# nash169/manifold-gp

Hardware: AMD Instinct MI355X
Metric: CG-solve wall-time + SpMV HBM GB/s, N=60k RMNIST graph (higher is better)
Workload: dtype f32; 1 GPU; C3 RMNIST-like N=60000 d=784 k=50 nu=2 randomwalk; nodes=60000, edges=1777442, nnz_padded=3667592, rhs_columns=1, system=A = I + noise*outputscale*Q, Q=(2nu/kappa^2 I + L)^nu x D, solver=CG on A (Chronopoulos-Gear, one hipGraph per solve)

## Files before the change

### include/mgp_hip.h

```cpp
#ifndef MGP_HIP_H
#define MGP_HIP_H

#include <stddef.h>
#include <stdint.h>

#ifdef __cplusplus
extern "C" {
#endif

#define MGP_OK 0
#define MGP_ERR_ARG (-1)
#define MGP_ERR_WORKSPACE (-2)
#define MGP_ERR_UNSUPPORTED (-3)
#define MGP_ERR_NOT_CONVERGED (-4)
#define MGP_ERR_KNN_AMBIGUOUS (-5)
#define MGP_ERR_TIMEOUT (-6)

#define MGP_PAD 4

int mgp_version(void);
int mgp_device_info(int* cu_count, int* wave_size, size_t* hbm_bytes);

size_t mgp_knn_workspace_bytes(int64_t N, int64_t n, int d, int k);
int mgp_knn_search(const float* db, int64_t N, int d, const float* q, int64_t n, int k,
// ... 46 lines not shown
int mgp_spmm_backward_sums(int64_t n, int C, const float* h, const float* dlx, const float* xs, const float* gxs, const float* X,
                           const float* g, const float* lx, float av, float bv, float cov, float* partial, float* gpre,
                           float* gpost, void* stream);
int mgp_edge_values(const int32_t* tri_row, const int32_t* tri_col, const float* tri_val,
                    int64_t M, const float* degree_unnorm, const float* degree, float eps,
                    int which, float* out, void* stream);

typedef struct {
  int64_t n;
  const int32_t* rowptr;
  const int32_t* col;
  const float* vals;
  const float* diag;
  int64_t ncols;
  const int32_t* tile_ptr;
  const int32_t* tile_cols;
  const uint16_t* lid;
  int32_t tile_rows;
  int32_t tile_max_cols;
  int32_t tile_max_entries;
  int32_t spmv_lanes;
  const int32_t* tile_rowptr;
  const float* tile_vals;
  const int32_t* tile_rowid;
  const int32_t* mt_sptr;
  const int32_t* mt_dcol;
  const float* mt_img;
  int32_t mt_tiles;
  int32_t mt_steps;
} mgp_csr_t;

int mgp_spmm_dot_blocks_csr(const mgp_csr_t* L, int C);
int mgp_spmm_set_tile_mode(int on);
int mgp_spmm_set_tile_small_mode(int on);
int mgp_spmm_set_tile_wide_mode(int on);
int mgp_spmm_set_dict_mode(int on);
int mgp_spmm_set_mt_mode(int on);
int mgp_spmm_kernel_choice(const mgp_csr_t* L, int C, int with_dot, int64_t row_offset);
int mgp_spmm_mt_fill(int64_t n, const int32_t* rowptr, const float* vals, const uint16_t* lid16, const int32_t* tile_ptr16,
                     const int32_t* tile_cols16, const int32_t* sptr, int64_t steps, int32_t* dcol, float* img, void* stream);
int mgp_spmm_timing_begin(int max_launches);
int mgp_spmm_timing_end(float* total_ms, int* launches);
int mgp_spmm_set_v4_mode(int on);

int mgp_spmm_dot_blocks(int64_t n, int C);
int mgp_spmm_set_group_hint(int lanes);
int mgp_spmm_set_rows_in_flight(int rows);
int mgp_spmm_fused(const mgp_csr_t* L, const float* X, int C, float* Y, float a, float b,
                   const float* pre, const float* post, const float* base, float cb, float co,
                   const float* dotw, float* dot_partials, void* stream);

int mgp_spmm_fused_rows(const mgp_csr_t* L_local, int64_t row_offset, const float* X, int C, float* Y,
                        float a, float b, const float* pre, const float* post, const float* base,
                        float cb, float co, const float* dotw, float* dot_partials, void* stream);

int mgp_spmm_repeat(const mgp_csr_t* L, const float* X, int C, float* Y, int reps, float* elapsed_ms,
                    void* stream);

int mgp_laplacian_matmul(const mgp_csr_t* L, const float* dsqrt, const float* dinvsqrt, int mode,
                         const float* X, int C, float* Y, float* work_nc, void* stream);

int mgp_gmrf_noise(const mgp_csr_t* L, const float* dsqrt, float node_coef, int tag, int with_edges,
                   uint64_t seed, int64_t sample_offset, int S, float* Y, void* stream);

typedef struct {
  mgp_csr_t L;
// ... 189 lines not shown
```

### manifold_gp_amd/_lib.py

```python
import ctypes
import os
import threading
from ctypes import (POINTER, Structure, byref, c_double, c_float, c_int, c_int32, c_int64, c_size_t,
                    c_uint64, c_void_p)

import torch

_HERE = os.path.dirname(os.path.abspath(__file__))
LIB_PATH = os.path.join(_HERE, "libmgp_hip.so")
_LIB = None
_LOCK = threading.Lock()

MGP_ERRORS = {
    -1: "MGP_ERR_ARG (null pointer / bad size / bad enum)",
    -2: "MGP_ERR_WORKSPACE (work buffer too small)",
    -3: "MGP_ERR_UNSUPPORTED",
    -4: "MGP_ERR_NOT_CONVERGED",
    -5: "MGP_ERR_KNN_AMBIGUOUS",
}


class MgpError(RuntimeError):
    def __init__(self, fn, code):
        self.code = code
# ... 26 lines not shown
class LanczosParamsT(Structure):
    _fields_ = [("max_basis", c_int32), ("degree", c_int32), ("max_restarts", c_int32),
                ("tol", c_float), ("seed", c_uint64)]


_P = c_void_p
SIGNATURES = {
    "mgp_version": (c_int, []),
    "mgp_device_info": (c_int, [POINTER(c_int), POINTER(c_int), POINTER(c_size_t)]),
    "mgp_knn_workspace_bytes": (c_size_t, [c_int64, c_int64, c_int, c_int]),
    "mgp_knn_search": (c_int, [_P, c_int64, c_int, _P, c_int64, c_int, _P, _P, _P, c_size_t,
                               POINTER(c_int64), _P]),
    "mgp_knn_set_mfma": (c_int, [c_int]),
    "mgp_knn_set_symmetric": (c_int, [c_int]),
    "mgp_knn_set_filter": (c_int, [c_int]),
    "mgp_knn_last_filter_failover": (c_int64, []),
    "mgp_knn_index_bytes": (c_size_t, [c_int64, c_int]),
    "mgp_knn_index_build": (c_int, [_P, c_int64, c_int, _P, c_size_t, _P]),
    "mgp_knn_search_indexed": (c_int, [_P, c_int64, c_int, _P, c_size_t, _P, c_int64, c_int, _P, _P, _P, c_size_t, _P, _P]),
    "mgp_knn_last_direct_chunks": (c_int64, []),
    "mgp_graph_workspace_bytes": (c_size_t, [c_int64, c_int]),
    "mgp_graph_edges": (c_int, [_P, _P, c_int64, c_int, c_int, c_int, _P, _P, _P, POINTER(c_int64), _P, c_size_t, _P]),
    "mgp_graph_tiles_workspace_bytes": (c_size_t, [c_int64, c_int64]),
    "mgp_graph_tiles": (c_int, [c_int64, _P, _P, c_int64, c_int, _P, _P, _P, _P, _P, _P, POINTER(c_int64),
                                POINTER(c_int32), POINTER(c_int32), _P, c_size_t, _P]),
    "mgp_morton_order_workspace_bytes": (c_size_t, [c_int64]),
    "mgp_morton_order": (c_int, [_P, c_int64, c_int, _P, _P, c_size_t, _P]),
    "mgp_graph_chain_order": (c_int, [c_int64, _P, _P, _P, _P, _P]),
    "mgp_permute_rows": (c_int, [_P, _P, c_int64, c_int, _P, _P]),
    "mgp_graph_bfs_workspace_bytes": (c_size_t, [c_int64]),
    "mgp_graph_bfs_order": (c_int, [c_int64, _P, _P, _P, _P, c_size_t, _P]),
    "mgp_spmm_dot_blocks_csr": (c_int, [POINTER(CsrT), c_int]),
    "mgp_spmm_set_tile_mode": (c_int, [c_int]),
    "mgp_spmm_set_tile_small_mode": (c_int, [c_int]),
    "mgp_spmm_set_tile_wide_mode": (c_int, [c_int]),
    "mgp_spmm_set_dict_mode": (c_int, [c_int]),
    "mgp_spmm_set_mt_mode": (c_int, [c_int]),
    "mgp_spmm_kernel_choice": (c_int, [POINTER(CsrT), c_int, c_int, c_int64]),
    "mgp_spmm_mt_fill": (c_int, [c_int64, _P, _P, _P, _P, _P, _P, c_int64, _P, _P, _P]),
    "mgp_spmm_timing_begin": (c_int, [c_int]),
    "mgp_spmm_timing_end": (c_int, [POINTER(c_float), POINTER(c_int)]),
    "mgp_spmm_set_v4_mode": (c_int, [c_int]),
    "mgp_cg_set_decide_in_update": (c_int, [c_int]),
    "mgp_cg_set_complex_shift": (c_int, [c_int]),
    "mgp_cg_plan_is_complex_shift": (c_int, [_P]),
    "mgp_cg_set_fold_update": (c_int, [c_int]),
    "mgp_cg_plan_is_folded": (c_int, [_P]),
    "mgp_cg_set_reduce_once": (c_int, [c_int]),
    "mgp_cg_set_update_quads": (c_int, [c_int]),
    "mgp_cg_set_poll_spin": (c_int, [c_int]),
    "mgp_cg_set_init_free": (c_int, [c_int]),
    "mgp_host_symeig": (c_int, [c_int, _P, _P, _P]),
    "mgp_lanczos_set_bound_mode": (c_int, [c_int]),
    "mgp_blz_workspace_bytes": (c_size_t, [c_int64, c_int, c_int]),
    "mgp_blz_begin": (c_int, [_P, c_int64, c_int, c_int, _P, c_size_t, _P]),
    "mgp_blz_q": (c_void_p, [c_int64, c_int, c_int, c_int, _P, c_size_t]),
    "mgp_blz_step": (c_int, [_P, c_int64, c_int, c_int, c_int, _P, c_size_t, _P]),
    "mgp_blz_end": (c_int, [c_int64, c_int, c_int, POINTER(c_float), POINTER(c_float), _P, c_size_t, _P]),
    "mgp_lanczos_tridiag_block_workspace_bytes": (c_size_t, [POINTER(OperatorT), c_int, c_int]),
    "mgp_lanczos_tridiag_block": (c_int, [POINTER(OperatorT), _P, c_int, c_int, POINTER(c_float), POINTER(c_float), _P,
                                         c_size_t, _P]),
    "mgp_graph_build": (c_int, [_P, _P, c_int64, c_int, _P, _P, _P, POINTER(c_int64), _P, _P, _P, _P,
                                POINTER(c_int64), _P, c_size_t, _P]),
    "mgp_graph_coo_workspace_bytes": (c_size_t, [c_int64, c_int64]),
    "mgp_graph_from_coo": (c_int, [_P, _P, _P, c_int64, c_int64, _P, _P, _P, _P, POINTER(c_int64), _P,
                                   c_size_t, _P]),
# ... 211 lines not shown
```

### manifold_gp_amd/csrc/spmm.hip

```cpp
#include <string.h>
#include <atomic>
#include <type_traits>
#include "mgp_common.h"
#include "mgp_internal.h"
#include "cg_rule.h"
#include "cg_handoff.h"
#include <hip/hip_ext.h>
#include <vector>

namespace {

constexpr int kBlock = 256;
constexpr int kMaxGrid = 4096;

struct SpmmArgs {
  int64_t n;
  const int32_t* rowptr;
  const int32_t* col;
  const float* vals;
  const float* diag;
  const float* X;
  float* Y;
  int C;
  float a, b;
// ... 128 lines not shown
      p.Y[myr + p.goff] = y;
      dsum = fmaf(e_dotw, y, dsum);
    }
  }
  if (p.dot_partials) {
    __shared__ float red[BS / MGP_WAVE];
    dsum = mgp_wave_sum(dsum);
    if ((threadIdx.x & 63) == 0) red[threadIdx.x >> 6] = dsum;
    __syncthreads();
    if (threadIdx.x == 0) {
      float t = 0.f;
#pragma unroll
      for (int w = 0; w < BS / MGP_WAVE; ++w) t += red[w];
      p.dot_partials[lb] = t;
    }
  }
}

struct TileArgs {
  const int32_t* tile_ptr;
  const int32_t* tile_cols;
  const uint16_t* lid;
  int64_t ntiles;
  int tiles_per_block;
  int max_cols;
  const int32_t* rowptr_t;
  const float* vals_t;
  const int32_t* rowid;
  int max_entries;
  int part_window;
};

typedef unsigned short mgp_v4h __attribute__((ext_vector_type(4)));

enum { kTilePlain = 0, kTileSelfDot = 1, kTileCgStep = 2 };
struct NoCgStep {};

template <bool PRE, int BS, bool CBV, int MODE, bool DECIDE, int DS, class CS>
__device__ __forceinline__ void spmv_tile_body(const SpmmArgs p, const TileArgs t, const CS cs) {
  extern __shared__ __attribute__((aligned(16))) float tile_lds[];
  const int lane0 = __builtin_amdgcn_mbcnt_lo(0u, 0u);
  const int* __restrict__ skip_ptr = (p.skip ? p.skip : reinterpret_cast<const int*>(p.rowptr)) + lane0;
  const int* __restrict__ tick_ptr = (p.tick ? p.tick : reinterpret_cast<const int*>(p.rowptr)) + lane0;
  int skipl = 0, tickl = 0;
  constexpr int TR = BS / 4;
  constexpr int NQ = 4;
  const int lb = mgp_xcd_block(blockIdx.x, gridDim.x);
  const int tid = threadIdx.x, sub = tid & 3;
#ifdef MGP_STAMP
  int* st_base = !p.stamp_on ? nullptr : (p.skip ? const_cast<int*>(p.skip) - 1 : p.tick);
  if (st_base && blockIdx.x == 0 && tid == 0) {
    const int si = atomicAdd(st_base + 8, 1);
    reinterpret_cast<unsigned long long*>(st_base + 16)[si & 255] = wall_clock64() * 8 + 0;
  }
  if (st_base && tid == 0 && blockIdx.x < 2048) reinterpret_cast<unsigned long long*>(st_base + 16)[256 + 2 * blockIdx.x] = wall_clock64();
#endif
  float* __restrict__ xl = tile_lds;
  float* __restrict__ part = tile_lds + t.max_cols;
  const float* __restrict__ x = p.X;
  const float* __restrict__ prev = p.pre;
  const int32_t* __restrict__ rowptr = t.rowptr_t ? t.rowptr_t : p.rowptr;
  const float* __restrict__ vals = t.vals_t ? t.vals_t : p.vals;
  const int32_t* __restrict__ tile_ptr = t.tile_ptr;
  const uint32_t* __restrict__ tile_cols = reinterpret_cast<const uint32_t*>(t.tile_cols);
  const uint16_t* __restrict__ lid = t.lid;
  float dsum = 0.f, dsum2 = 0.f;
  const int64_t t0 = (int64_t)lb * t.tiles_per_block;
  const int64_t t1 = t0 + t.tiles_per_block < t.ntiles ? t0 + t.tiles_per_block : t.ntiles;
  __shared__ float cg_sh_w[MODE == kTileCgStep ? BS / MGP_WAVE : 1][3];
  __shared__ float cg_sh_o[MODE == kTileCgStep ? BS / MGP_WAVE : 1];
  __shared__ int cg_sh_state[MODE == kTileCgStep ? 2 : 1];
  __shared__ int cg_sh_last[1];
  [[maybe_unused]] float cg_rv[2][DS], cg_dv[DS];
  [[maybe_unused]] float cg_go0 = 0.f, cg_go1 = 0.f, cg_ao0 = 0.f, cg_ao1 = 0.f, cg_bb_old = 0.f;
  [[maybe_unused]] int cg_st_it = 0, cg_st_done = 0;
  [[maybe_unused]] float cg_alpha = 0.f, cg_beta = 0.f, cg_bb = 0.f, cg_nrr = 0.f;
  [[maybe_unused]] int cg_it = 0;
  [[maybe_unused]] bool cg_fresh = false;
  if constexpr (MODE == kTileCgStep) {
    static_assert(BS == 256, "the step's sums are written for four waves");
    const CgScalars sc = *reinterpret_cast<const CgScalars*>(cs.blk);
    cg_go0 = sc.go0; cg_go1 = sc.go1; cg_ao0 = sc.ao0; cg_ao1 = sc.ao1; cg_bb_old = sc.bb; cg_st_it = sc.it; cg_st_done = sc.done;
#pragma unroll
    for (int q = 0; q < DS; ++q) {
      const int b = tid + q * BS;
      const int bc = b < cs.nbs ? b : cs.nbs - 1;
      cg_rv[0][q] = cs.pd_rr[bc];
      cg_rv[1][q] = cs.pd_rr[cs.nbs + bc];
      cg_dv[q] = cs.pd_delta[bc];
    }
  }
  for (int64_t tile = t0; tile < t1; ++tile) {
    skipl = *skip_ptr;
    tickl = *tick_ptr;
    const int64_t r0 = tile * TR;
    const int64_t r1 = r0 + TR < p.n ? r0 + TR : p.n;
    const int e0 = rowptr[r0], e1 = rowptr[r1];
    const int dp = tile_ptr[tile];
    const int D = tile_ptr[tile + 1] - dp;
    const int qb = e0 >> 2, Q = (e1 - e0) >> 2;
    unsigned c[NQ];
#pragma unroll
    for (int k = 0; k < NQ; ++k) {
      const int j = tid + k * BS;
      c[k] = (unsigned)tile_cols[j < D ? dp + j : 0];
    }
    __builtin_amdgcn_sched_barrier(0);
    mgp_v4f v[NQ];
    mgp_v4h l[NQ];
#pragma unroll
    for (int k = 0; k < NQ / 2; ++k) {
      const int q = tid + k * BS;
      const int qi = q < Q ? qb + q : 0;
      v[k] = *reinterpret_cast<const mgp_v4f*>(vals + 4 * (int64_t)qi);
      l[k] = *reinterpret_cast<const mgp_v4h*>(lid + 4 * (int64_t)qi);
    }
    __builtin_amdgcn_sched_barrier(0);
    float g[NQ];
#pragma unroll
    for (int k = 0; k < NQ; ++k) {
      g[k] = x[c[k]];
      if (PRE) g[k] *= prev[c[k]];
    }
    __builtin_amdgcn_sched_barrier(0);
#pragma unroll
    for (int k = NQ / 2; k < NQ; ++k) {
      const int q = tid + k * BS;
      const int qi = q < Q ? qb + q : 0;
      v[k] = *reinterpret_cast<const mgp_v4f*>(vals + 4 * (int64_t)qi);
      l[k] = *reinterpret_cast<const mgp_v4h*>(lid + 4 * (int64_t)qi);
    }
    __builtin_amdgcn_sched_barrier(0);
    const int64_t row = r0 + (tid >> 2);
    const bool valid = row < r1;
    const int64_t pr = valid ? row : r0;
    const int64_t rr = t.rowid ? (int64_t)t.rowid[pr] : pr;
    const int64_t grr = rr + p.goff;
    const int rs = rowptr[pr], re = rowptr[pr + 1];
    const float raw_x = x[grr];
    float e_x = raw_x;
    if (PRE) e_x *= prev[grr];
    const float e_diag = p.diag[rr];
    const float l_post = (p.post ? p.post : x)[grr], l_base = (p.base ? p.base : x)[grr], l_dotw = (p.dotw ? p.dotw : x)[grr];
    const float e_post = p.post ? l_post : 1.f;
    const float e_base = p.base ? l_base : 0.f;
    const float e_dotw = p.dotw ? l_dotw : 0.f;
    const float e_cb = CBV ? p.cbv[grr] : p.cb;
    [[maybe_unused]] float f_r = 0.f, f_s = 0.f, f_p = 0.f, f_x = 0.f, f_pre = 1.f;
    if constexpr (MODE == kTileCgStep) {
      f_r = cs.r[grr]; f_s = cs.s[grr]; f_p = cs.p[grr]; f_x = cs.x[grr];
      const float l_pre = (cs.us ? cs.pre : x)[grr];
      f_pre = cs.us ? l_pre : 1.f;
    }
    __builtin_amdgcn_sched_barrier(0);
    if (p.skip && skipl) return;
    if constexpr (MODE == kTileCgStep) {
      if (tile == t0) {
        float s3[3] = {0.f, 0.f, 0.f};
#pragma unroll
        for (int q = 0; q < DS; ++q) {
          const bool on = tid + q * BS < cs.nbs;
          s3[0] += on ? cg_rv[0][q] : 0.f; s3[1] += on ? cg_rv[1][q] : 0.f; s3[2] += on ? cg_dv[q] : 0.f;
        }
#pragma unroll
        for (int k = 0; k < 3; ++k) s3[k] = mgp_wave_sum(s3[k]);
        if ((tid & 63) == 0) {
#pragma unroll
          for (int k = 0; k < 3; ++k) cg_sh_w[tid >> 6][k] = s3[k];
        }
        if (tid == 0) { cg_sh_state[0] = cg_st_it; cg_sh_state[1] = cg_st_done; }
      }
    }
#pragma unroll
    for (int k = 0; k < NQ; ++k) {
      const int j = tid + k * BS;
      if (j < D) xl[j] = g[k];
    }
    for (int j = tid + NQ * BS; j < D; j += BS) {
      const int cc = tile_cols[dp + j];
      float gg = x[cc];
      if (PRE) gg *= prev[cc];
      xl[j] = gg;
    }
    __syncthreads();
    if constexpr (MODE == kTileCgStep) {
      if (tile == t0) {
        const int it = cg_sh_state[0];
        const bool fresh = it == 1;
        auto zero_x = [&]() {
          for (int64_t tl = t0; tl < t1; ++tl) {
            const int64_t pos = tl * TR + tid;
            if (tid < TR && pos < p.n) cs.x[t.rowid ? (int64_t)t.rowid[pos] : pos] = 0.f;
          }
        };
        if (cg_sh_state[1]) {
          if (fresh) zero_x();
          if (DECIDE && blockIdx.x == 0 && tid == 0) cg_mark_end_of_graph(cs.state, cs.host_state);
          return;
        }
        const int par = it & 1, prev = par ^ 1;
        float tt3[3];
#pragma unroll
        for (int k = 0; k < 3; ++k) tt3[k] = (cg_sh_w[0][k] + cg_sh_w[1][k]) + (cg_sh_w[2][k] + cg_sh_w[3][k]);
        const float rr2 = prev ? tt3[1] : tt3[0];
        const float gamma = rr2;
        const float delta = (cs.dgamma ? gamma : 0.f) + cs.dcoef * tt3[2];
        const float bb = (it == 1) ? rr2 : cg_bb_old;
        const float rel = cg_rel(rr2, bb);
        const CgCoef kc = cg_coef(it == 1, cg_frozen(cs.stop_mode, cs.tol, rel), gamma, delta, prev ? cg_go1 : cg_go0,
                                  prev ? cg_ao1 : cg_ao0);
        const CgStop st = cg_stop(cs.stop_mode, cs.min_iter, cs.max_iter, cs.tol, it, rel);
        if (blockIdx.x == 0 && tid == 0) {
          float* gamma_old = cs.blk;
          float* alpha_old = cs.blk + 2;
          gamma_old[par] = gamma;
          alpha_old[par] = kc.alpha;
          if (it == 1) cs.blk[4] = bb;
          if (!DECIDE || st.done) cs.blk[5] = rel;
          if (st.done) cg_publish(cs.state, cs.host_state, cs.host_resid, &rel, 1, it, st.status);
        }
        if (st.done) {
          if (fresh) zero_x();
          if (DECIDE && blockIdx.x == 0 && tid == 0) cg_mark_end_of_graph(cs.state, cs.host_state);
          return;
        }
        cg_alpha = kc.alpha; cg_beta = kc.beta; cg_bb = bb; cg_it = it; cg_fresh = fresh;
      }
    }
#pragma unroll
    for (int k = 0; k < NQ; ++k) {
      const int q = tid + k * BS;
      if (q < Q) {
        float s = v[k].x * xl[l[k].x];
        s = fmaf(v[k].y, xl[l[k].y], s);
        s = fmaf(v[k].z, xl[l[k].z], s);
        s = fmaf(v[k].w, xl[l[k].w], s);
        part[q] = s;
      }
    }
    for (int q = tid + NQ * BS; q < Q; q += BS) {
      const mgp_v4f vv = *reinterpret_cast<const mgp_v4f*>(vals + 4 * (int64_t)(qb + q));
      const mgp_v4h ll = *reinterpret_cast<const mgp_v4h*>(lid + 4 * (int64_t)(qb + q));
      float s = vv.x * xl[ll.x];
      s = fmaf(vv.y, xl[ll.y], s);
      s = fmaf(vv.z, xl[ll.z], s);
      s = fmaf(vv.w, xl[ll.w], s);
      part[q] = s;
    }
    __syncthreads();
    float acc = 0.f;
    {
      int i = (rs >> 2) - qb + sub;
      const int e = (re >> 2) - qb;
      for (; i + 12 < e; i += 16) {
        const float a0 = part[i], a1 = part[i + 4], a2 = part[i + 8], a3 = part[i + 12];
        acc += a0; acc += a1; acc += a2; acc += a3;
      }
      for (; i < e; i += 4) acc += part[i];
    }
    acc = mgp_quad_sum(acc);
    if (valid && sub == 0) {
      const float lx = e_diag * e_x - acc;
      const float tt = (p.a * e_x + p.b * lx) * e_post;
      if constexpr (MODE == kTileCgStep) {
        const float w = p.co * tt + (cs.dgamma ? e_cb * f_r : 0.f);
        const float po = cg_fresh ? 0.f : f_p, so = cg_fresh ? 0.f : f_s, xo = cg_fresh ? 0.f : f_x;
        const float pn = fmaf(cg_beta, po, f_r);
        const float sn = fmaf(cg_beta, so, w);
        cs.p[grr] = pn;
        cs.s[grr] = sn;
        cs.x[grr] = fmaf(cg_alpha, pn, xo);
        const float rn = fmaf(-cg_alpha, sn, f_r);
        cs.r[grr] = rn;
        if (cs.us) cs.us[grr] = f_pre * rn;
        cg_nrr = fmaf(rn, rn, cg_nrr);
      } else {
        const float y = p.co * tt + e_cb * e_base;
        p.Y[grr] = y;
        if constexpr (MODE == kTileSelfDot) {
          dsum = fmaf(y, y, dsum);
          dsum2 = fmaf(raw_x, raw_x, dsum2);
        } else {
// ... 15 lines not shown
    if constexpr (DECIDE) {
      const CgHandoff h{cs.arrive, cs.state, cs.host_state, cs.blk + 5, cs.tol, cs.max_iter, cs.min_iter, cs.stop_mode};
      cg_handoff_decide<DS>(h, rr_par, cs.nbs, lb, o_r, cg_it, cg_bb, cg_sh_o, cg_sh_last);
    } else if (tid == 0) rr_par[lb] = o_r;
    return;
  }
  if (p.tick && blockIdx.x == 0 && tid == 0 && !(p.skip && skipl)) {
    if (p.tick_reset) { p.tick[0] = 1; p.tick[1] = 0; p.tick[2] = 0; }
    else *p.tick = tickl + 1;
  }
  if (p.dot_partials) {
    __shared__ float red[2][BS / MGP_WAVE];
    dsum = mgp_wave_sum(dsum);
    if (p.dot2_partials) dsum2 = mgp_wave_sum(dsum2);
    if ((tid & 63) == 0) { red[0][tid >> 6] = dsum; red[1][tid >> 6] = dsum2; }
    __syncthreads();
    if (tid == 0) {
      float s = 0.f, s2 = 0.f;
#pragma unroll
      for (int w = 0; w < BS / MGP_WAVE; ++w) { s += red[0][w]; s2 += red[1][w]; }
      p.dot_partials[lb] = s;
      if (p.dot2_partials) p.dot2_partials[lb] = s2;
    }
  }
#ifdef MGP_STAMP
  if (st_base && blockIdx.x == 0 && tid == 0) {
    const int si = atomicAdd(st_base + 8, 1);
    reinterpret_cast<unsigned long long*>(st_base + 16)[si & 255] = wall_clock64() * 8 + 1;
  }
  if (st_base && tid == 0 && blockIdx.x < 2048) reinterpret_cast<unsigned long long*>(st_base + 16)[256 + 2 * blockIdx.x + 1] = wall_clock64();
#endif
}

template <bool PRE, int BS, bool CBV, bool SELF>
__global__ __launch_bounds__(BS) void spmv_tile_kernel(SpmmArgs p, TileArgs t) {
  spmv_tile_body<PRE, BS, CBV, SELF ? kTileSelfDot : kTilePlain, false, 1>(p, t, NoCgStep{});
}

template <int BS, int DS, bool DECIDE>
__global__ __launch_bounds__(BS) void spmv_tile_cgstep_kernel(SpmmArgs p, TileArgs t, MgpCgStep cs) {
  spmv_tile_body<false, BS, false, kTileCgStep, DECIDE, DS>(p, t, cs);
}

template <int G, int NACC, bool PRE, bool CBV>
__global__ __launch_bounds__(kBlock) void spmm_kernel(SpmmArgs p) {
  if (p.skip && *p.skip) return;
  if (p.tick && blockIdx.x == 0 && threadIdx.x == 0) *p.tick += 1;
  const int lb = mgp_xcd_block(blockIdx.x, gridDim.x);
  const int lane = threadIdx.x & (G - 1);
  const int grp = threadIdx.x / G;
  constexpr int kGroups = kBlock / G;
  const int C = p.C;
  const int64_t r0 = (int64_t)lb * p.rows_per_block;
  int64_t r1 = r0 + p.rows_per_block;
  if (r1 > p.n) r1 = p.n;
  float dsum[NACC];
#pragma unroll
  for (int a = 0; a < NACC; ++a) dsum[a] = 0.f;

  for (int64_t r = r0 + grp; r < r1; r += kGroups) {
    const int s = p.rowptr[r], e = p.rowptr[r + 1];
    float acc[NACC];
#pragma unroll
    for (int a = 0; a < NACC; ++a) acc[a] = 0.f;
    for (int i0 = s; i0 < e; i0 += G) {
      const int i = i0 + lane;
      int cj = (int)(r + p.goff);
      float vj = 0.f;
      if (i < e) { cj = p.col[i]; vj = p.vals[i]; }
      if (PRE) vj *= p.pre[cj];
      const int cnt = (e - i0) < G ? (e - i0) : G;
      constexpr int U = G >= 8 ? 8 : G;
      for (int t0 = 0; t0 < cnt; t0 += U) {
        float vts[U];
// ... 830 lines not shown
    }
  }
  const int d0 = tile_ptr[t], D = tile_ptr[t + 1] - d0;
  const int total = 4 * (sptr[t + 1] - (int)s0);
  for (int q = i; q < total; q += 16) dcol[4 * s0 + q] = D > 0 ? tile_cols[d0 + (q < D ? q : D - 1)] : 0;
}

struct SpmvTimer {
  std::vector<hipEvent_t> ev;
  int used = 0;
  bool on = false;
};
SpmvTimer g_spmv_timer;

struct Plan {
  int grid;
  int64_t rows_per_block;
};

Plan make_plan(int64_t n, int rows_per_pass) {
  int64_t rpb = rows_per_pass;
  int64_t grid = mgp_cdiv(n, rpb);
  if (grid > kMaxGrid) {
    rpb = mgp_cdiv(mgp_cdiv(n, kMaxGrid), rows_per_pass) * rows_per_pass;
    grid = mgp_cdiv(n, rpb);
  }
  if (grid < 1) grid = 1;
  return Plan{(int)grid, rpb};
}

std::atomic<int> g_row_group_hint{16};
std::atomic<int> g_rows_in_flight{1};
std::atomic<int> g_tile_mode{1};
std::atomic<int> g_tile_small_mode{1};
std::atomic<int> g_tile_wide_mode{1};
std::atomic<int> g_spmm_v4_mode{1};
std::atomic<int> g_dict_mode{1};
std::atomic<int> g_mt_mode{1};
#ifdef MGP_STAMP
std::atomic<int> g_stamp_enable{0};
#endif

}

extern "C" int mgp_spmm_set_group_hint(int lanes) {
  if (!mgp_spmv_lanes_ok(lanes) || lanes == 0) return MGP_ERR_ARG;
  g_row_group_hint = lanes;
  return MGP_OK;
}

extern "C" int mgp_spmm_set_rows_in_flight(int rows) {
  if (rows != 1 && rows != 2 && rows != 4 && rows != 8) return MGP_ERR_ARG;
  g_rows_in_flight = rows;
  return MGP_OK;
}

#ifdef MGP_STAMP
extern "C" int mgp_stamp_enable(int on) { g_stamp_enable = on ? 1 : 0; return 0; }
#endif

extern "C" int mgp_spmm_set_tile_mode(int on) {
  g_tile_mode = on ? 1 : 0;
  return MGP_OK;
}

extern "C" int mgp_spmm_set_v4_mode(int on) {
  g_spmm_v4_mode = on == 2 ? 2 : (on ? 1 : 0);
  return MGP_OK;
}

extern "C" int mgp_spmm_set_tile_wide_mode(int on) {
  g_tile_wide_mode = on == 2 ? 2 : (on ? 1 : 0);
  return MGP_OK;
}

extern "C" int mgp_spmm_set_tile_small_mode(int on) {
  g_tile_small_mode = on ? 1 : 0;
  return MGP_OK;
}

extern "C" int mgp_spmm_set_dict_mode(int on) {
  g_dict_mode = on == 2 ? 2 : (on ? 1 : 0);
  return MGP_OK;
}

extern "C" int mgp_spmm_set_mt_mode(int on) {
  const int prev = g_mt_mode;
  g_mt_mode = on ? 1 : 0;
  return prev;
}

#ifdef MGP_MT_STAMP
extern "C" int mgp_mt_set_stamp_buffer(void* buf) {
  g_mt_stamps = static_cast<unsigned long long*>(buf);
  return MGP_OK;
// ... 86 lines not shown
  const int64_t ntiles = mgp_cdiv(L->n, L->tile_rows);
  return (int)(ntiles < kMaxGrid ? ntiles : kMaxGrid);
}

constexpr int kMtMinCols = 48;
static bool mt_image_fits(const mgp_csr_t* L, int C) {
  if (!L->mt_img || !L->mt_sptr || !L->mt_dcol || L->mt_tiles <= 0 || L->mt_steps <= 0) return false;
  if (C < kMtMinCols || C > 256 || (C & 3) != 0 || L->tile_rowid) return false;
  if (L->ncols != 0 && L->ncols != L->n) return false;
  if ((int64_t)L->n * C * 4 >= (int64_t(1) << 31) || ((int64_t)L->mt_steps + 32) * 256 >= (int64_t(1) << 31)) return false;
  if ((L->mt_steps & 15) != 0) return false;
  return L->mt_tiles == (int32_t)mgp_cdiv(L->n, 16);
}

static TileArgs tile_args(const mgp_csr_t* L, int tiles_per_block, int part_window) {
  return TileArgs{L->tile_ptr, L->tile_cols, L->lid, mgp_cdiv(L->n, L->tile_rows), tiles_per_block, L->tile_max_cols,
                  L->tile_rowptr, L->tile_vals, L->tile_rowid, L->tile_max_entries, part_window};
}

namespace {
enum class SpmmFamily { RowGroups, Gather, TileC1, TileSmall, MatrixCore, Dict, TileWide };

struct SpmmPlan {
  int err;
  SpmmFamily family;
  int grid;
  size_t lds;
  int dot_blocks;
  bool align16;
  int64_t rows_per_block;
  int lanes, rows_in_flight;
  bool v4_ok;
  int tiles_per_block;
  int window;
  int slots, stream_cap;
  int wide_cap;
};
}

static SpmmPlan spmm_plan(const mgp_csr_t* L, int C, int64_t row_offset, bool with_dot) {
  SpmmPlan pl{};
  pl.tiles_per_block = 1;
  if (!mgp_spmv_lanes_ok(L->spmv_lanes)) { pl.err = MGP_ERR_ARG; return pl; }
  const int tile = g_tile_mode, tile_small = g_tile_small_mode, tile_wide = g_tile_wide_mode, v4 = g_spmm_v4_mode,
            dict = g_dict_mode, mt = g_mt_mode;
  const int ord = (L->tile_rowptr != nullptr) + (L->tile_vals != nullptr) + (L->tile_rowid != nullptr);
  const bool dicts = tile && (ord == 0 || ord == 3) && L->lid && L->tile_ptr && L->tile_cols;
  const bool dicts64 = dicts && L->tile_rows == 64 && (L->tile_max_entries & 3) == 0;
  const bool wide = C > 16 && C <= 256 && (C & 3) == 0;
  const bool big_x = (size_t)L->n * (size_t)C * sizeof(float) >= ((size_t)96 << 20);

  if (C == 1 && dicts && (L->tile_rows == 32 || L->tile_rows == 64 || L->tile_rows == 128) && tile_lds_bytes(L) <= 65536 - 64) {
    pl.family = SpmmFamily::TileC1;
    pl.grid = pl.dot_blocks = tile_grid(L, &pl.tiles_per_block);
    pl.lds = tile_lds_bytes(L);
    return pl;
  }
  if ((C == 4 || C == 8 || C == 12 || C == 16) && tile_small && dicts64 && tile_small_lds_bytes(L, C) <= 65536 - 64) {
    pl.family = SpmmFamily::TileSmall;
    pl.align16 = true;
    pl.grid = pl.dot_blocks = tile_grid(L, &pl.tiles_per_block);
    pl.lds = tile_small_lds_bytes(L, C);
    pl.window = tile_small_window(L);
    return pl;
  }
  if (mt && mt_image_fits(L, C)) {
    if (row_offset == 0) {
      pl.family = SpmmFamily::MatrixCore;
      pl.align16 = true;
      pl.grid = pl.dot_blocks = (int)mgp_cdiv((int64_t)L->mt_tiles * ((C + 63) / 64), kBlock / 64);
      return pl;
    }
    if (with_dot) { pl.err = MGP_ERR_UNSUPPORTED; return pl; }
  }
  if (wide && dict && dicts64 && dict_slots(L, C) >= 32 && (dict == 2 || (C >= 64 && big_x))) {
    pl.family = SpmmFamily::Dict;
    pl.align16 = true;
    pl.grid = pl.dot_blocks = dict_grid(L);
    pl.lds = dict_lds_bytes(L, C);
    pl.slots = dict_slots(L, C);
    pl.stream_cap = dict_stream_cap(L);
    return pl;
  }
  if (wide && tile_wide && dicts64 && (tile_wide == 2 || big_x)) {
    pl.family = SpmmFamily::TileWide;
    pl.align16 = true;
    pl.grid = pl.dot_blocks = tile_grid(L, &pl.tiles_per_block);
// ... 99 lines not shown
  MGP_HIP_TRY(hipGraphExecKernelNodeSetParams(static_cast<hipGraphExec_t>(exec), static_cast<hipGraphNode_t>(node), &np));
  return MGP_OK;
}

namespace {
template <int V> using IntC = std::integral_constant<int, V>;
template <class F> static void with_pre(bool pre, F&& f) { if (pre) f(std::true_type{}); else f(std::false_type{}); }
template <class F> static void with_quads(int C, F&& f) {
  if (C == 4) f(IntC<1>{});
  else if (C == 8) f(IntC<2>{});
  else if (C == 12) f(IntC<3>{});
  else f(IntC<4>{});
}

static bool aligned16(const void* a, const void* b, const void* c = nullptr, const void* d = nullptr) {
  return ((reinterpret_cast<uintptr_t>(a) | reinterpret_cast<uintptr_t>(b) | reinterpret_cast<uintptr_t>(c) |
           reinterpret_cast<uintptr_t>(d)) & 15) == 0;
}

template <bool CB>
int spmm_launch(const SpmmPlan& pl, const mgp_csr_t* L, void* record_to, SpmmArgs& p, hipStream_t st, bool self_dot = false) {
  const int C = p.C, grid = pl.grid;
  const size_t lds = pl.lds;
  const bool pre = p.pre != nullptr;
  if (pl.align16 && !aligned16(p.X, p.Y, p.base, p.dotw)) return MGP_ERR_ARG;
  p.rows_per_block = pl.rows_per_block;
  switch (pl.family) {
  case SpmmFamily::TileC1: {
    TileArgs ta = tile_args(L, pl.tiles_per_block, 0);
    if (record_to) {
      TileLaunchRecord rec{p, ta};
      memcpy(record_to, &rec, sizeof(rec));
    }
    auto tiles = [&](auto bs) { with_pre(pre, [&](auto P) {
      constexpr int BS = decltype(bs)::value;
      const auto kernel = self_dot ? &spmv_tile_kernel<decltype(P)::value, BS, CB, true> : &spmv_tile_kernel<decltype(P)::value, BS, CB, false>;
      if (g_spmv_timer.on && 2 * g_spmv_timer.used + 1 < (int)g_spmv_timer.ev.size()) {
        hipEvent_t e0 = g_spmv_timer.ev[2 * g_spmv_timer.used], e1 = g_spmv_timer.ev[2 * g_spmv_timer.used + 1];
        ++g_spmv_timer.used;
        hipExtLaunchKernelGGL(kernel, dim3(grid), dim3(BS), lds, st, e0, e1, 0, p, ta);
      } else hipLaunchKernelGGL(kernel, dim3(grid), dim3(BS), lds, st, p, ta);
    }); };
    if (L->tile_rows == 32) tiles(IntC<128>{});
    else if (L->tile_rows == 64) tiles(IntC<256>{});
    else tiles(IntC<512>{});
  } break;
  case SpmmFamily::TileSmall: {
    TileArgs ta = tile_args(L, pl.tiles_per_block, pl.window);
    with_quads(C, [&](auto c4) { with_pre(pre, [&](auto P) {
      hipLaunchKernelGGL((spmm_tile_q_kernel<decltype(c4)::value, decltype(P)::value, CB>), dim3(grid), dim3(256), lds, st, p, ta);
    }); });
  } break;
  case SpmmFamily::MatrixCore: {
    MtArgs ma{L->mt_sptr, L->mt_dcol, L->mt_img, L->mt_tiles, (C + 63) / 64, (int)(((int64_t)L->mt_steps + 32) * 256),
              (int)(((int64_t)L->mt_steps * 4 + 192) * 4)};
#if defined(MGP_MT_LAB) && (MGP_MT_LAB & 1)
    ma.img_bytes = 0;
#endif
#ifdef MGP_MT_STAMP
    ma.stamps = g_mt_stamps;
#endif
    with_pre(pre, [&](auto P) {
      if constexpr (CB) hipLaunchKernelGGL((spmm_mt_cbv_kernel<decltype(P)::value>), dim3(grid), dim3(kBlock), 0, st, p, ma);
      else hipLaunchKernelGGL((spmm_mt_kernel<decltype(P)::value>), dim3(grid), dim3(kBlock), 0, st, p, ma);
    });
  } break;
  case SpmmFamily::Dict: {
    TileArgs ta = tile_args(L, 1, 0);
    const int S = pl.slots, cap = pl.stream_cap;
    hipError_t attr = hipSuccess;
    auto slices = [&](auto nv) { with_pre(pre, [&](auto P) {
      const auto kernel = &spmm_dict_kernel<decltype(nv)::value, decltype(P)::value, CB>;
      attr = hipFuncSetAttribute(reinterpret_cast<const void*>(kernel), hipFuncAttributeMaxDynamicSharedMemorySize, kDictLdsBudget);
      if (attr == hipSuccess) hipLaunchKernelGGL(kernel, dim3(grid), dim3(kDictThreads), lds, st, p, ta, S, cap);
    }); };
    switch (dict_nv(C)) {
      case 1: slices(IntC<1>{}); break;
      case 2: slices(IntC<2>{}); break;
// ... 69 lines not shown
  const SpmmPlan pl = spmm_plan(L, C, o.row_offset, (dotw || self_dot) && dot_partials);
  if (pl.err != MGP_OK) return pl.err;
  if (o.self_dot && (pl.family != SpmmFamily::TileC1 || dotw || o.cbv || !dot_partials)) return MGP_ERR_UNSUPPORTED;
  SpmmArgs p{L->n, L->rowptr, L->col, L->vals, L->diag, X, Y, C, a, b, pre, post, base, cb, co,
             dotw, (dotw || self_dot) ? dot_partials : nullptr, 0, o.skip, o.tick, o.row_offset, nullptr, nullptr, 0, o.cbv};
#ifdef MGP_STAMP
  p.stamp_on = g_stamp_enable;
#endif
  if (o.first) {
    if (pl.family != SpmmFamily::TileC1) return MGP_ERR_UNSUPPORTED;
    p.copy_x = o.first->copy_x;
    p.dot2_partials = ((dotw || self_dot) && dot_partials) ? o.first->dot2_partials : nullptr;
    p.tick_reset = o.first->tick_reset;
  }
  void* record_to = o.first ? o.first->record : nullptr;
  hipStream_t st = mgp_stream(stream);
  return o.cbv ? spmm_launch<true>(pl, L, record_to, p, st) : spmm_launch<false>(pl, L, record_to, p, st, self_dot);
}

int mgp_spmm_cgstep(const mgp_csr_t* L, const float* T, float a, float b, const float* post, float co, const MgpCgStep& cs,
                    bool decide, void* stream) {
  if (!L || !L->rowptr || !L->col || !L->vals || !L->diag || !T || L->n <= 0) return MGP_ERR_ARG;
  if (!cs.r || !cs.x || !cs.p || !cs.s || !cs.pd_rr || !cs.pd_delta || !cs.blk || !cs.state || !cs.host_state || !cs.host_resid ||
      !cs.arrive || (cs.us && !cs.pre) || T == cs.r || T == cs.us) return MGP_ERR_ARG;
  const SpmmPlan pl = spmm_plan(L, 1, 0, true);
  if (pl.err != MGP_OK) return pl.err;
  if (pl.family != SpmmFamily::TileC1 || L->tile_rows != 64 || pl.lds + kCgStepStaticLds > 65536) return MGP_ERR_UNSUPPORTED;
  if (cs.nbs != pl.dot_blocks || cs.nbs < 1 || cs.nbs > 16 * 256) return MGP_ERR_ARG;
  SpmmArgs p{L->n, L->rowptr, L->col, L->vals, L->diag, T, nullptr, 1, a, b, nullptr, post, nullptr, 1.f, co,
             nullptr, nullptr, 0, nullptr, nullptr, 0, nullptr, nullptr, 0, nullptr};
  const TileArgs ta = tile_args(L, pl.tiles_per_block, 0);
  const dim3 grid(pl.grid), block(256);
  hipStream_t st = mgp_stream(stream);
  if (cs.nbs <= 4 * 256) {
    if (decide) hipLaunchKernelGGL((spmv_tile_cgstep_kernel<256, 4, true>), grid, block, pl.lds, st, p, ta, cs);
    else hipLaunchKernelGGL((spmv_tile_cgstep_kernel<256, 4, false>), grid, block, pl.lds, st, p, ta, cs);
  } else {
    if (decide) hipLaunchKernelGGL((spmv_tile_cgstep_kernel<256, 16, true>), grid, block, pl.lds, st, p, ta, cs);
    else hipLaunchKernelGGL((spmv_tile_cgstep_kernel<256, 16, false>), grid, block, pl.lds, st, p, ta, cs);
  }
  MGP_LAUNCH_CHECK();
  return MGP_OK;
}

extern "C" int mgp_spmm_fused(const mgp_csr_t* L, const float* X, int C, float* Y, float a, float b,
                              const float* pre, const float* post, const float* base, float cb,
                              float co, const float* dotw, float* dot_partials, void* stream) {
  return mgp_spmm_fused_opts(L, X, C, Y, a, b, pre, post, base, cb, co, dotw, dot_partials, MgpSpmmOpts{}, stream);
}

__global__ void scale_rows_kernel(const float* __restrict__ s, const float* __restrict__ x,
                                  float* __restrict__ y, int64_t n, int C) {
  int64_t total = n * C;
  for (int64_t i = blockIdx.x * (int64_t)blockDim.x + threadIdx.x; i < total;
       i += (int64_t)gridDim.x * blockDim.x)
    y[i] = s[i / C] * x[i];
}

extern "C" int mgp_laplacian_matmul(const mgp_csr_t* L, const float* dsqrt, const float* dinvsqrt,
                                    int mode, const float* X, int C, float* Y, float* work_nc,
                                    void* stream) {
  (void)work_nc;
  if (mode < 0 || mode > 2) return MGP_ERR_ARG;
  if (mode != 0 && (!dsqrt || !dinvsqrt)) return MGP_ERR_ARG;
  const float* pre = mode == 0 ? nullptr : (mode == 1 ? dsqrt : dinvsqrt);
  const float* post = mode == 0 ? nullptr : (mode == 1 ? dinvsqrt : dsqrt);
  return mgp_spmm_fused(L, X, C, Y, 0.f, 1.f, pre, post, nullptr, 0.f, 1.f, nullptr, nullptr, stream);
}

extern "C" int mgp_spmm_fused_rows(const mgp_csr_t* L_local, int64_t row_offset, const float* X, int C, float* Y,
                                   float a, float b, const float* pre, const float* post, const float* base,
                                   float cb, float co, const float* dotw, float* dot_partials, void* stream) {
  if (row_offset < 0) return MGP_ERR_ARG;
// ... 70 lines not shown
```

Measured before the change: 3567 GB/s (algorithmic SpMV bytes inside the CG solve).

## Specialize tile SpMV for one tile per block and defer CG partial reads

Adds a compile-time ONE variant of the tile SpMV and CG-step kernels for the case where each block handles exactly one tile, which removes the tile loop bounds and per-tile skip/tick loads. It forces kernel arguments into scalar registers at kernel entry with an inline-asm hint, loads the CG scalar block as a single 8-int vector, and, for small partial counts, moves the partial-sum reads and reduction past the x gather so they overlap with the SpMV work. The intent is to shorten the kernel prologue and hide latency in the CG step. In exchange it adds template variants and a tile-loop mode switch, and relies on scheduling barriers and asm constraints that could raise scalar register pressure.

```diff
diff --git a/include/mgp_hip.h b/include/mgp_hip.h
--- a/include/mgp_hip.h
+++ b/include/mgp_hip.h
@@ -102,6 +102,7 @@
 
 int mgp_spmm_dot_blocks_csr(const mgp_csr_t* L, int C);
 int mgp_spmm_set_tile_mode(int on);
+int mgp_spmm_set_tile_loop_mode(int on);
 int mgp_spmm_set_tile_small_mode(int on);
 int mgp_spmm_set_tile_wide_mode(int on);
 int mgp_spmm_set_dict_mode(int on);
diff --git a/manifold_gp_amd/_lib.py b/manifold_gp_amd/_lib.py
--- a/manifold_gp_amd/_lib.py
+++ b/manifold_gp_amd/_lib.py
@@ -82,6 +82,7 @@
     "mgp_graph_bfs_order": (c_int, [c_int64, _P, _P, _P, _P, c_size_t, _P]),
     "mgp_spmm_dot_blocks_csr": (c_int, [POINTER(CsrT), c_int]),
     "mgp_spmm_set_tile_mode": (c_int, [c_int]),
+    "mgp_spmm_set_tile_loop_mode": (c_int, [c_int]),
     "mgp_spmm_set_tile_small_mode": (c_int, [c_int]),
     "mgp_spmm_set_tile_wide_mode": (c_int, [c_int]),
     "mgp_spmm_set_dict_mode": (c_int, [c_int]),
diff --git a/manifold_gp_amd/csrc/spmm.hip b/manifold_gp_amd/csrc/spmm.hip
--- a/manifold_gp_amd/csrc/spmm.hip
+++ b/manifold_gp_amd/csrc/spmm.hip
@@ -184,23 +184,61 @@
 };
 
 typedef unsigned short mgp_v4h __attribute__((ext_vector_type(4)));
+typedef int mgp_v8i __attribute__((ext_vector_type(8)));
 
 enum { kTilePlain = 0, kTileSelfDot = 1, kTileCgStep = 2 };
 struct NoCgStep {};
 
-template <bool PRE, int BS, bool CBV, int MODE, bool DECIDE, int DS, class CS>
-__device__ __forceinline__ void spmv_tile_body(const SpmmArgs p, const TileArgs t, const CS cs) {
+template <bool STEP>
+struct TileView {
+  int64_t n, goff;
+  const int32_t* rowptr;
+  const float *vals, *diag, *X, *pre, *post, *base, *dotw, *cbv;
+  float *Y, *dot_partials, *copy_x, *dot2_partials;
+  float a, b, cb, co;
+  const int* skip;
+  int* tick;
+  int tick_reset;
+  __device__ __forceinline__ explicit TileView(const SpmmArgs& p)
+      : n(p.n), goff(STEP ? 0 : p.goff), rowptr(p.rowptr), vals(p.vals), diag(p.diag), X(p.X), pre(STEP ? nullptr : p.pre),
+        post(p.post), base(STEP ? nullptr : p.base), dotw(STEP ? nullptr : p.dotw), cbv(STEP ? nullptr : p.cbv),
+        Y(STEP ? nullptr : p.Y), dot_partials(STEP ? nullptr : p.dot_partials), copy_x(STEP ? nullptr : p.copy_x),
+        dot2_partials(STEP ? nullptr : p.dot2_partials), a(p.a), b(p.b), cb(p.cb), co(p.co), skip(STEP ? nullptr : p.skip),
+        tick(STEP ? nullptr : p.tick), tick_reset(STEP ? 0 : p.tick_reset) {}
+};
+
+template <bool PRE, int BS, bool CBV, int MODE, bool DECIDE, int DS, bool ONE, class CS>
+__device__ __forceinline__ void spmv_tile_body(const SpmmArgs pa, const TileArgs t, const CS cs) {
   extern __shared__ __attribute__((aligned(16))) float tile_lds[];
-  const int lane0 = __builtin_amdgcn_mbcnt_lo(0u, 0u);
-  const int* __restrict__ skip_ptr = (p.skip ? p.skip : reinterpret_cast<const int*>(p.rowptr)) + lane0;
-  const int* __restrict__ tick_ptr = (p.tick ? p.tick : reinterpret_cast<const int*>(p.rowptr)) + lane0;
+  constexpr bool STEP = MODE == kTileCgStep;
+  const TileView<STEP> p(pa);
+  int zero;
+  const unsigned grid_x = gridDim.x;
+#define MGP_TILE_HEAD_ARGS                                                                                                     \
+  "s"(p.n), "s"(p.rowptr), "s"(t.rowptr_t), "s"(p.vals), "s"(t.vals_t), "s"(p.diag), "s"(p.X), "s"(p.post), "s"(p.a), "s"(p.b),   \
+      "s"(p.cb), "s"(p.co), "s"(t.tile_ptr), "s"(t.tile_cols), "s"(t.lid), "s"(t.max_cols), "s"(t.rowid), "s"(grid_x),           \
+      "s"(PRE ? p.pre : nullptr), "s"(CBV ? p.cbv : nullptr), "s"(ONE ? (int64_t)0 : t.ntiles), "s"(ONE ? 0 : t.tiles_per_block)
+  if constexpr (!STEP) {
+    asm("s_mov_b32 %0, 0" : "=s"(zero) : MGP_TILE_HEAD_ARGS, "s"(p.goff), "s"(p.base), "s"(p.dotw), "s"(p.Y), "s"(p.dot_partials),
+        "s"(p.copy_x), "s"(p.dot2_partials), "s"(p.skip), "s"(p.tick), "s"(p.tick_reset));
+  } else {
+    asm("s_mov_b32 %0, 0" : "=s"(zero) : MGP_TILE_HEAD_ARGS, "s"(cs.r), "s"(cs.x), "s"(cs.p), "s"(cs.s), "s"(cs.us), "s"(cs.pre),
+        "s"(cs.pd_rr), "s"(cs.pd_delta), "s"(cs.nbs), "s"(cs.blk), "s"(cs.state), "s"(cs.host_state), "s"(cs.host_resid),
+        "s"(cs.arrive), "s"(cs.tol), "s"(cs.max_iter), "s"(cs.min_iter), "s"(cs.stop_mode), "s"(cs.dcoef), "s"(cs.dgamma));
+  }
+#undef MGP_TILE_HEAD_ARGS
+  const int32_t* __restrict__ rowptr = t.rowptr_t ? t.rowptr_t : p.rowptr;
+  const float* __restrict__ vals = t.vals_t ? t.vals_t : p.vals;
+  const int lane0 = __builtin_amdgcn_mbcnt_lo(0u, 0u) + zero;
+  const int* __restrict__ skip_ptr = (p.skip ? p.skip : reinterpret_cast<const int*>(rowptr)) + lane0;
+  const int* __restrict__ tick_ptr = (p.tick ? p.tick : reinterpret_cast<const int*>(rowptr)) + lane0;
   int skipl = 0, tickl = 0;
   constexpr int TR = BS / 4;
   constexpr int NQ = 4;
-  const int lb = mgp_xcd_block(blockIdx.x, gridDim.x);
+  const int lb = mgp_xcd_block(blockIdx.x, grid_x) + zero;
   const int tid = threadIdx.x, sub = tid & 3;
 #ifdef MGP_STAMP
-  int* st_base = !p.stamp_on ? nullptr : (p.skip ? const_cast<int*>(p.skip) - 1 : p.tick);
+  int* st_base = !pa.stamp_on ? nullptr : (p.skip ? const_cast<int*>(p.skip) - 1 : p.tick);
   if (st_base && blockIdx.x == 0 && tid == 0) {
     const int si = atomicAdd(st_base + 8, 1);
     reinterpret_cast<unsigned long long*>(st_base + 16)[si & 255] = wall_clock64() * 8 + 0;
@@ -211,46 +249,80 @@
   float* __restrict__ part = tile_lds + t.max_cols;
   const float* __restrict__ x = p.X;
   const float* __restrict__ prev = p.pre;
-  const int32_t* __restrict__ rowptr = t.rowptr_t ? t.rowptr_t : p.rowptr;
-  const float* __restrict__ vals = t.vals_t ? t.vals_t : p.vals;
   const int32_t* __restrict__ tile_ptr = t.tile_ptr;
   const uint32_t* __restrict__ tile_cols = reinterpret_cast<const uint32_t*>(t.tile_cols);
   const uint16_t* __restrict__ lid = t.lid;
   float dsum = 0.f, dsum2 = 0.f;
-  const int64_t t0 = (int64_t)lb * t.tiles_per_block;
-  const int64_t t1 = t0 + t.tiles_per_block < t.ntiles ? t0 + t.tiles_per_block : t.ntiles;
+  const int64_t t0 = ONE ? (int64_t)lb : (int64_t)lb * t.tiles_per_block;
+  const int64_t t1 = ONE ? t0 + 1 : (t0 + t.tiles_per_block < t.ntiles ? t0 + t.tiles_per_block : t.ntiles);
   __shared__ float cg_sh_w[MODE == kTileCgStep ? BS / MGP_WAVE : 1][3];
   __shared__ float cg_sh_o[MODE == kTileCgStep ? BS / MGP_WAVE : 1];
   __shared__ int cg_sh_state[MODE == kTileCgStep ? 2 : 1];
   __shared__ int cg_sh_last[1];
-  [[maybe_unused]] float cg_rv[2][DS], cg_dv[DS];
+  constexpr bool CG_LATE = DS <= 4;
+  [[maybe_unused]] float cg_rv[2][DS], cg_dv[DS], cg_s3[3] = {0.f, 0.f, 0.f};
+  [[maybe_unused]] auto cg_request_partials = [&]() {
+    if constexpr (STEP) {
+#pragma unroll
+      for (int q = 0; q < DS; ++q) {
+        const int b = tid + q * BS;
+        const int bc = b < cs.nbs ? b : cs.nbs - 1;
+        cg_rv[0][q] = cs.pd_rr[bc];
+        cg_rv[1][q] = cs.pd_rr[cs.nbs + bc];
+        cg_dv[q] = cs.pd_delta[bc];
+      }
+    }
+  };
+  [[maybe_unused]] auto cg_sum_partials = [&]() {
+    if constexpr (STEP) {
+#pragma unroll
+      for (int q = 0; q < DS; ++q) {
+        const bool on = tid + q * BS < cs.nbs;
+        cg_s3[0] += on ? cg_rv[0][q] : 0.f; cg_s3[1] += on ? cg_rv[1][q] : 0.f; cg_s3[2] += on ? cg_dv[q] : 0.f;
+      }
+#pragma unroll
+      for (int k = 0; k < 3; ++k) cg_s3[k] = mgp_wave_sum(cg_s3[k]);
+    }
+  };
   [[maybe_unused]] float cg_go0 = 0.f, cg_go1 = 0.f, cg_ao0 = 0.f, cg_ao1 = 0.f, cg_bb_old = 0.f;
   [[maybe_unused]] int cg_st_it = 0, cg_st_done = 0;
+  [[maybe_unused]] mgp_v8i cg_blk;
+  [[maybe_unused]] auto take_blk = [&]() {
+    asm("" : "+s"(cg_blk));
+    const CgScalars sc = __builtin_bit_cast(CgScalars, cg_blk);
+    cg_go0 = sc.go0; cg_go1 = sc.go1; cg_ao0 = sc.ao0; cg_ao1 = sc.ao1; cg_bb_old = sc.bb; cg_st_it = sc.it; cg_st_done = sc.done;
+  };
   [[maybe_unused]] float cg_alpha = 0.f, cg_beta = 0.f, cg_bb = 0.f, cg_nrr = 0.f;
   [[maybe_unused]] int cg_it = 0;
   [[maybe_unused]] bool cg_fresh = false;
   if constexpr (MODE == kTileCgStep) {
     static_assert(BS == 256, "the step's sums are written for four waves");
-    const CgScalars sc = *reinterpret_cast<const CgScalars*>(cs.blk);
-    cg_go0 = sc.go0; cg_go1 = sc.go1; cg_ao0 = sc.ao0; cg_ao1 = sc.ao1; cg_bb_old = sc.bb; cg_st_it = sc.it; cg_st_done = sc.done;
-#pragma unroll
-    for (int q = 0; q < DS; ++q) {
-      const int b = tid + q * BS;
-      const int bc = b < cs.nbs ? b : cs.nbs - 1;
-      cg_rv[0][q] = cs.pd_rr[bc];
-      cg_rv[1][q] = cs.pd_rr[cs.nbs + bc];
-      cg_dv[q] = cs.pd_delta[bc];
-    }
-  }
+    static_assert(sizeof(CgScalars) == sizeof(mgp_v8i) && alignof(CgScalars) == alignof(mgp_v8i), "the scalar block is one load");
+    cg_blk = *reinterpret_cast<const mgp_v8i*>(cs.blk);
+    if constexpr (!ONE) take_blk();
+    if constexpr (!CG_LATE) { cg_request_partials(); cg_sum_partials(); }
+  }
+  [[maybe_unused]] auto zero_x = [&]() {
+    if constexpr (STEP) {
+      for (int64_t tl = t0; tl < t1; ++tl) {
+        const int64_t pos = tl * TR + tid;
+        if (tid < TR && pos < p.n) cs.x[t.rowid ? (int64_t)t.rowid[pos] : pos] = 0.f;
+      }
+    }
+  };
   for (int64_t tile = t0; tile < t1; ++tile) {
-    skipl = *skip_ptr;
-    tickl = *tick_ptr;
+    if constexpr (!STEP) {
+      skipl = *skip_ptr;
+      tickl = *tick_ptr;
+    }
     const int64_t r0 = tile * TR;
     const int64_t r1 = r0 + TR < p.n ? r0 + TR : p.n;
     const int e0 = rowptr[r0], e1 = rowptr[r1];
     const int dp = tile_ptr[tile];
     const int D = tile_ptr[tile + 1] - dp;
     const int qb = e0 >> 2, Q = (e1 - e0) >> 2;
+    __builtin_amdgcn_sched_barrier(0);
+    if constexpr (STEP && ONE) take_blk();
     unsigned c[NQ];
 #pragma unroll
     for (int k = 0; k < NQ; ++k) {
@@ -308,18 +380,8 @@
     if (p.skip && skipl) return;
     if constexpr (MODE == kTileCgStep) {
       if (tile == t0) {
-        float s3[3] = {0.f, 0.f, 0.f};
-#pragma unroll
-        for (int q = 0; q < DS; ++q) {
-          const bool on = tid + q * BS < cs.nbs;
-          s3[0] += on ? cg_rv[0][q] : 0.f; s3[1] += on ? cg_rv[1][q] : 0.f; s3[2] += on ? cg_dv[q] : 0.f;
-        }
-#pragma unroll
-        for (int k = 0; k < 3; ++k) s3[k] = mgp_wave_sum(s3[k]);
-        if ((tid & 63) == 0) {
-#pragma unroll
-          for (int k = 0; k < 3; ++k) cg_sh_w[tid >> 6][k] = s3[k];
-        }
+        if constexpr (CG_LATE) cg_request_partials();
+        __builtin_amdgcn_sched_barrier(0);
         if (tid == 0) { cg_sh_state[0] = cg_st_it; cg_sh_state[1] = cg_st_done; }
       }
     }
@@ -337,19 +399,44 @@
     __syncthreads();
     if constexpr (MODE == kTileCgStep) {
       if (tile == t0) {
-        const int it = cg_sh_state[0];
-        const bool fresh = it == 1;
-        auto zero_x = [&]() {
-          for (int64_t tl = t0; tl < t1; ++tl) {
-            const int64_t pos = tl * TR + tid;
-            if (tid < TR && pos < p.n) cs.x[t.rowid ? (int64_t)t.rowid[pos] : pos] = 0.f;
-          }
-        };
+        cg_it = cg_sh_state[0];
+        cg_fresh = cg_it == 1;
         if (cg_sh_state[1]) {
-          if (fresh) zero_x();
+          if (cg_fresh) zero_x();
           if (DECIDE && blockIdx.x == 0 && tid == 0) cg_mark_end_of_graph(cs.state, cs.host_state);
           return;
         }
+        if constexpr (CG_LATE) cg_sum_partials();
+        if ((tid & 63) == 0) {
+#pragma unroll
+          for (int k = 0; k < 3; ++k) cg_sh_w[tid >> 6][k] = cg_s3[k];
+        }
+      }
+    }
+#pragma unroll
+    for (int k = 0; k < NQ; ++k) {
+      const int q = tid + k * BS;
+      if (q < Q) {
+        float s = v[k].x * xl[l[k].x];
+        s = fmaf(v[k].y, xl[l[k].y], s);
+        s = fmaf(v[k].z, xl[l[k].z], s);
+        s = fmaf(v[k].w, xl[l[k].w], s);
+        part[q] = s;
+      }
+    }
+    for (int q = tid + NQ * BS; q < Q; q += BS) {
+      const mgp_v4f vv = *reinterpret_cast<const mgp_v4f*>(vals + 4 * (int64_t)(qb + q));
+      const mgp_v4h ll = *reinterpret_cast<const mgp_v4h*>(lid + 4 * (int64_t)(qb + q));
+      float s = vv.x * xl[ll.x];
+      s = fmaf(vv.y, xl[ll.y], s);
+      s = fmaf(vv.z, xl[ll.z], s);
+      s = fmaf(vv.w, xl[ll.w], s);
+      part[q] = s;
+    }
+    __syncthreads();
+    if constexpr (MODE == kTileCgStep) {
+      if (tile == t0) {
+        const int it = cg_it;
         const int par = it & 1, prev = par ^ 1;
         float tt3[3];
 #pragma unroll
@@ -372,34 +459,13 @@
           if (st.done) cg_publish(cs.state, cs.host_state, cs.host_resid, &rel, 1, it, st.status);
         }
         if (st.done) {
-          if (fresh) zero_x();
+          if (cg_fresh) zero_x();
           if (DECIDE && blockIdx.x == 0 && tid == 0) cg_mark_end_of_graph(cs.state, cs.host_state);
           return;
         }
-        cg_alpha = kc.alpha; cg_beta = kc.beta; cg_bb = bb; cg_it = it; cg_fresh = fresh;
-      }
-    }
-#pragma unroll
-    for (int k = 0; k < NQ; ++k) {
-      const int q = tid + k * BS;
-      if (q < Q) {
-        float s = v[k].x * xl[l[k].x];
-        s = fmaf(v[k].y, xl[l[k].y], s);
-        s = fmaf(v[k].z, xl[l[k].z], s);
-        s = fmaf(v[k].w, xl[l[k].w], s);
-        part[q] = s;
-      }
-    }
-    for (int q = tid + NQ * BS; q < Q; q += BS) {
-      const mgp_v4f vv = *reinterpret_cast<const mgp_v4f*>(vals + 4 * (int64_t)(qb + q));
-      const mgp_v4h ll = *reinterpret_cast<const mgp_v4h*>(lid + 4 * (int64_t)(qb + q));
-      float s = vv.x * xl[ll.x];
-      s = fmaf(vv.y, xl[ll.y], s);
-      s = fmaf(vv.z, xl[ll.z], s);
-      s = fmaf(vv.w, xl[ll.w], s);
-      part[q] = s;
-    }
-    __syncthreads();
+        cg_alpha = kc.alpha; cg_beta = kc.beta; cg_bb = bb;
+      }
+    }
     float acc = 0.f;
     {
       int i = (rs >> 2) - qb + sub;
@@ -481,14 +547,14 @@
 #endif
 }
 
-template <bool PRE, int BS, bool CBV, bool SELF>
+template <bool PRE, int BS, bool CBV, bool SELF, bool ONE>
 __global__ __launch_bounds__(BS) void spmv_tile_kernel(SpmmArgs p, TileArgs t) {
-  spmv_tile_body<PRE, BS, CBV, SELF ? kTileSelfDot : kTilePlain, false, 1>(p, t, NoCgStep{});
-}
-
-template <int BS, int DS, bool DECIDE>
+  spmv_tile_body<PRE, BS, CBV, SELF ? kTileSelfDot : kTilePlain, false, 1, ONE>(p, t, NoCgStep{});
+}
+
+template <int BS, int DS, bool DECIDE, bool ONE>
 __global__ __launch_bounds__(BS) void spmv_tile_cgstep_kernel(SpmmArgs p, TileArgs t, MgpCgStep cs) {
-  spmv_tile_body<false, BS, false, kTileCgStep, DECIDE, DS>(p, t, cs);
+  spmv_tile_body<false, BS, false, kTileCgStep, DECIDE, DS, ONE>(p, t, cs);
 }
 
 template <int G, int NACC, bool PRE, bool CBV>
@@ -1385,6 +1451,7 @@
 std::atomic<int> g_row_group_hint{16};
 std::atomic<int> g_rows_in_flight{1};
 std::atomic<int> g_tile_mode{1};
+std::atomic<int> g_tile_loop_mode{0};
 std::atomic<int> g_tile_small_mode{1};
 std::atomic<int> g_tile_wide_mode{1};
 std::atomic<int> g_spmm_v4_mode{1};
@@ -1414,6 +1481,11 @@
 
 extern "C" int mgp_spmm_set_tile_mode(int on) {
   g_tile_mode = on ? 1 : 0;
+  return MGP_OK;
+}
+
+extern "C" int mgp_spmm_set_tile_loop_mode(int on) {
+  g_tile_loop_mode = on ? 1 : 0;
   return MGP_OK;
 }
 
@@ -1566,6 +1638,7 @@
   int lanes, rows_in_flight;
   bool v4_ok;
   int tiles_per_block;
+  bool one_tile;
   int window;
   int slots, stream_cap;
   int wide_cap;
@@ -1587,6 +1660,7 @@
   if (C == 1 && dicts && (L->tile_rows == 32 || L->tile_rows == 64 || L->tile_rows == 128) && tile_lds_bytes(L) <= 65536 - 64) {
     pl.family = SpmmFamily::TileC1;
     pl.grid = pl.dot_blocks = tile_grid(L, &pl.tiles_per_block);
+    pl.one_tile = pl.tiles_per_block == 1 && !g_tile_loop_mode;
     pl.lds = tile_lds_bytes(L);
     return pl;
   }
@@ -1752,18 +1826,20 @@
       TileLaunchRecord rec{p, ta};
       memcpy(record_to, &rec, sizeof(rec));
     }
-    auto tiles = [&](auto bs) { with_pre(pre, [&](auto P) {
+    auto tiles = [&](auto bs, auto one) { with_pre(pre, [&](auto P) {
       constexpr int BS = decltype(bs)::value;
-      const auto kernel = self_dot ? &spmv_tile_kernel<decltype(P)::value, BS, CB, true> : &spmv_tile_kernel<decltype(P)::value, BS, CB, false>;
+      constexpr bool ONE = decltype(one)::value;
+      const auto kernel = self_dot ? &spmv_tile_kernel<decltype(P)::value, BS, CB, true, ONE> : &spmv_tile_kernel<decltype(P)::value, BS, CB, false, ONE>;
       if (g_spmv_timer.on && 2 * g_spmv_timer.used + 1 < (int)g_spmv_timer.ev.size()) {
         hipEvent_t e0 = g_spmv_timer.ev[2 * g_spmv_timer.used], e1 = g_spmv_timer.ev[2 * g_spmv_timer.used + 1];
         ++g_spmv_timer.used;
         hipExtLaunchKernelGGL(kernel, dim3(grid), dim3(BS), lds, st, e0, e1, 0, p, ta);
       } else hipLaunchKernelGGL(kernel, dim3(grid), dim3(BS), lds, st, p, ta);
     }); };
-    if (L->tile_rows == 32) tiles(IntC<128>{});
-    else if (L->tile_rows == 64) tiles(IntC<256>{});
-    else tiles(IntC<512>{});
+    auto forms = [&](auto bs) { if (pl.one_tile) tiles(bs, std::true_type{}); else tiles(bs, std::false_type{}); };
+    if (L->tile_rows == 32) forms(IntC<128>{});
+    else if (L->tile_rows == 64) forms(IntC<256>{});
+    else forms(IntC<512>{});
   } break;
   case SpmmFamily::TileSmall: {
     TileArgs ta = tile_args(L, pl.tiles_per_block, pl.window);
@@ -1899,13 +1975,14 @@
   const TileArgs ta = tile_args(L, pl.tiles_per_block, 0);
   const dim3 grid(pl.grid), block(256);
   hipStream_t st = mgp_stream(stream);
-  if (cs.nbs <= 4 * 256) {
-    if (decide) hipLaunchKernelGGL((spmv_tile_cgstep_kernel<256, 4, true>), grid, block, pl.lds, st, p, ta, cs);
-    else hipLaunchKernelGGL((spmv_tile_cgstep_kernel<256, 4, false>), grid, block, pl.lds, st, p, ta, cs);
-  } else {
-    if (decide) hipLaunchKernelGGL((spmv_tile_cgstep_kernel<256, 16, true>), grid, block, pl.lds, st, p, ta, cs);
-    else hipLaunchKernelGGL((spmv_tile_cgstep_kernel<256, 16, false>), grid, block, pl.lds, st, p, ta, cs);
-  }
+  auto step = [&](auto ds, auto one) {
+    constexpr int DS = decltype(ds)::value;
+    constexpr bool ONE = decltype(one)::value;
+    if (decide) hipLaunchKernelGGL((spmv_tile_cgstep_kernel<256, DS, true, ONE>), grid, block, pl.lds, st, p, ta, cs);
+    else hipLaunchKernelGGL((spmv_tile_cgstep_kernel<256, DS, false, ONE>), grid, block, pl.lds, st, p, ta, cs);
+  };
+  if (cs.nbs <= 4 * 256) { if (pl.one_tile) step(IntC<4>{}, std::true_type{}); else step(IntC<4>{}, std::false_type{}); }
+  else { if (pl.one_tile) step(IntC<16>{}, std::true_type{}); else step(IntC<16>{}, std::false_type{}); }
   MGP_LAUNCH_CHECK();
   return MGP_OK;
 }
```

Result: faster. 3925 GB/s (algorithmic SpMV bytes inside the CG solve) (median of 6 runs) (+10.0%).
